# It4innovations/hyperqueue

Measured on AMD Instinct MI355X. Metric: tasks_assigned_per_sec, higher is better.
Workload: dtype u64

## Files before the change

hyperqueue_amd/csrc/debug_capi.cpp:

```cpp
#include "../../include/hqtick_debug.h"

#include <algorithm>
#include <cstring>

#include "hb_order.h"
#include "milp.h"
#include "price_emul.h"

static thread_local int g_last_canonical = 0;
static thread_local long g_last_hull[2] = {0, 0};
extern "C" int hqtick_debug_milp_was_canonical(void) { return g_last_canonical; }
extern "C" void hqtick_debug_milp_last_hull(long *solves, long *nonpacking) {
    if (solves) *solves = g_last_hull[0];
    if (nonpacking) *nonpacking = g_last_hull[1];
}

extern "C" int hqtick_debug_milp_solve(int ncols, const double *obj, const uint8_t *col_kind, int nrows, const uint8_t *row_type,
                                       const double *rhs, const int *row_off, const int *row_col, const double *row_coef,
                                       double time_limit_s, int canonical, double *x_out, double *obj_out, int *is_optimal,
                                       long *nodes_out) {
    hqmilp::Model m;
    m.obj.assign(obj, obj + ncols);
    m.kind.assign(col_kind, col_kind + ncols);
    m.rtype.assign(row_type, row_type + nrows);
// ... 27 lines not shown
    m.kind.assign(col_kind, col_kind + ncols);
    m.rtype.assign(row_type, row_type + nrows);
    m.rhs.assign(rhs, rhs + nrows);
    m.roff.assign(row_off, row_off + nrows + 1);
    int nnz = nrows ? row_off[nrows] : 0;
    m.rcol.assign(row_col, row_col + nnz);
    m.rcoef.assign(row_coef, row_coef + nnz);
    if (col_group) m.col_group.assign(col_group, col_group + ncols);
    if (row_implied) m.row_implied.assign(row_implied, row_implied + nrows);
    hqprice::EmulatedSweeper emu;
    if (min_cols) emu.min_cols = min_cols;
    hqmilp::Result r = hqmilp::solve(m, time_limit_s, true, hqmilp::REFERENCE_MIP_REL_GAP, use_sweeps ? &emu : nullptr);
    g_last_canonical = r.canonical ? 1 : 0;
    g_last_hull[0] = r.hull_solves; g_last_hull[1] = r.hull_solves_nonpacking;
    if (stats_out) { stats_out[0] = r.price_sweeps; stats_out[1] = r.price_rounds; stats_out[2] = r.price_total_us; stats_out[3] = r.canonical ? 1.0 : 0.0; }
    if (!r.feasible) return 0;
    for (int j = 0; j < ncols; j++) x_out[j] = r.x[j];
    *obj_out = r.objective;
    *is_optimal = r.optimal ? 1 : 0;
    return 1;
}

static thread_local hqmilp::Probe g_block_run_probe;
extern "C" void hqtick_debug_set_block_runs(int on) {
    hqmilp::g_probe = on < 0 ? nullptr : &g_block_run_probe; hqmilp::set_block_runs(on);
    if (on >= 0) { g_block_run_probe.model = g_block_run_probe.tables = g_block_run_probe.runs = g_block_run_probe.covered = 0; }
}
extern "C" void hqtick_debug_corrupt_block_runs(int on) { g_block_run_probe.corrupt_runs = on != 0; }
extern "C" void hqtick_debug_last_coupled_digest(uint64_t out[4]) {
    out[0] = g_block_run_probe.model; out[1] = g_block_run_probe.tables; out[2] = g_block_run_probe.runs; out[3] = g_block_run_probe.covered;
}
extern "C" void hqtick_debug_set_early_sweep(int on) { hqprice::set_early_sweep(on); }
extern "C" uint32_t hqtick_debug_early_sweeps(void) { return hqprice::early_sweeps(); }
extern "C" void hqtick_debug_capture_first_cut(int on) { hqprice::capture_first_cut(on != 0); }
extern "C" uint32_t hqtick_debug_first_cut(unsigned char *out, uint32_t cap) {
    const std::vector<unsigned char> &b = hqprice::first_cut_bytes();
    if (out && cap) memcpy(out, b.data(), std::min<size_t>(cap, b.size()));
    return (uint32_t)b.size();
}
```

hyperqueue_amd/csrc/hqtick.cpp:

```cpp
#include "../../include/hqtick.h"
#ifdef HQTICK_TEST_HOOKS
#include "../../include/hqtick_debug.h"
#endif

#include <dlfcn.h>
#include <hip/hip_runtime.h>
#include <rccl/rccl.h>

#include <algorithm>
#include <chrono>
#include <cstdio>
#include <cstdlib>
#include <cstring>
#include <functional>
#include <map>
#include <string>
#include <vector>

#include "block_solve.h"
#include "price_dev.h"
#ifdef HQTICK_TEST_HOOKS
#include "price_emul.h"
#endif
#include "devbuf.h"
// ... 2763 lines not shown
int hqtick_shard_allgather(hqtick_ctx *ctx, void *recv_device, size_t recv_bytes) {
    if (!ctx || !recv_device) return HQTICK_E_INVALID;
    if (!ctx->comm) return fail(ctx, HQTICK_E_INVALID, "hqtick_shard_allgather without hqtick_comm_init");
    if (!ctx->sink || !ctx->sink_bytes) return fail(ctx, HQTICK_E_INVALID, "hqtick_shard_allgather without a record sink (hqtick_set_record_sink)");
    if (recv_bytes < (size_t)ctx->comm_world * ctx->sink_bytes) return fail(ctx, HQTICK_E_CAPACITY, "receive buffer smaller than world x sink bytes");
    HQ_HIP(hipSetDevice(ctx->device));
    ncclResult_t rc = rccl().all_gather(ctx->sink, recv_device, ctx->sink_bytes, ncclUint8, ctx->comm, ctx->stream);
    if (rc != ncclSuccess) return fail(ctx, HQTICK_E_DEVICE, std::string("ncclAllGather: ") + rccl().err(rc));
    HQ_HIP(hipStreamSynchronize(ctx->stream));
    return 0;
}

}

namespace {
bool rccl_allgather_host(hqtick_ctx *ctx, const void *send, void *recv, size_t bytes) {
    if (!ctx->comm || bytes == 0) return false;
    const size_t total = bytes * ctx->comm_world;
    if (!ctx->h_xsend.ensure(bytes) || !ctx->h_xrecv.ensure(total) || !ctx->d_xsend.ensure(bytes) || !ctx->d_xrecv.ensure(total)) return false;
    if (hipSetDevice(ctx->device) != hipSuccess) return false;
    memcpy(ctx->h_xsend.p, send, bytes);
    if (hipMemcpyAsync(ctx->d_xsend.p, ctx->h_xsend.p, bytes, hipMemcpyHostToDevice, ctx->stream) != hipSuccess) return false;
    if (rccl().all_gather(ctx->d_xsend.p, ctx->d_xrecv.p, bytes, ncclUint8, ctx->comm, ctx->stream) != ncclSuccess) return false;
    if (hipMemcpyAsync(ctx->h_xrecv.p, ctx->d_xrecv.p, total, hipMemcpyDeviceToHost, ctx->stream) != hipSuccess) return false;
    if (hipStreamSynchronize(ctx->stream) != hipSuccess) return false;
    memcpy(recv, ctx->h_xrecv.p, total);
    return true;
}
}

extern "C" {

#ifdef HQTICK_TEST_HOOKS
int hqtick_debug_exchange(hqtick_ctx *ctx, const void *send, void *recv, size_t bytes_per_rank) {
    if (!ctx || !send || !recv) return HQTICK_E_INVALID;
    if (!ctx->comm) return fail(ctx, HQTICK_E_INVALID, "hqtick_debug_exchange without hqtick_comm_init");
    return rccl_allgather_host(ctx, send, recv, bytes_per_rank) ? 0 : fail(ctx, HQTICK_E_DEVICE, "the RCCL exchange failed");
}
#endif

int hqtick_comm_destroy(hqtick_ctx *ctx) {
    if (!ctx) return HQTICK_E_INVALID;
    if (ctx->comm) { hipSetDevice(ctx->device); rccl().destroy(ctx->comm); ctx->comm = nullptr; }
    ctx->comm_world = 0; ctx->comm_rank = 0;
    return 0;
}

}

static void rccl_destroy_comm(hqtick_ctx *ctx) { hqtick_comm_destroy(ctx); }
```

hyperqueue_amd/csrc/price.cpp:

```cpp
#include "price.h"

#include <algorithm>
#include <chrono>
#include <cmath>
#include <cstdio>
#include <cstdlib>
#include <cstring>
#include <functional>
#include <map>
#include <numeric>

#include "lp_tab.h"
#include "milp.h"

namespace hqprice {
namespace {

using hqmilp::lp::BASIC;
using hqmilp::lp::INF;
using hqmilp::lp::LP_OPT;
using hqmilp::lp::Rows;
using hqmilp::lp::Tab;

constexpr int KMAX_HOST = 128;
// ... 1624 lines not shown
            const uint32_t b = (uint32_t)P.block_of_flat[f];
            const double *ba = &bact[(size_t)b * MMAX_BLOCK];
            for (int r = 0; r < (int)T.blk_m[b] && step >= 1.0; r++) { const double a = T.col_a[(size_t)f * MMAX_BLOCK + r]; if (a > 0.0) { const double room = T.blk_cap[(size_t)b * MMAX_BLOCK + r] - ba[r]; if (room < a) { step = 0.0; break; } step = std::min(step, std::floor(room / a + 1e-9)); } }
            for (uint32_t e = T.col_woff[f]; e < T.col_woff[f + 1] && step >= 1.0; e++) {
                const double a = (double)T.w_coef[e];
                if (!(a > 0.0)) continue;
                const int g = T.w_row[e];
                for (int q = P.gr_off[g]; q < P.gr_off[g + 1]; q++) { const int k = P.gr_row[q]; const double room = P.h[k] - (ga[g] + fl[k]); if (room < 0.5 * a) { step = 0.0; break; } step = std::min(step, std::floor(room / a + 1e-9)); }
            }
            if (step < 1.0) continue;
            xf[f] += step;
            double *bw = &bact[(size_t)b * MMAX_BLOCK];
            for (int r = 0; r < MMAX_BLOCK; r++) bw[r] += T.col_a[(size_t)f * MMAX_BLOCK + r] * step;
            for (uint32_t e = T.col_woff[f]; e < T.col_woff[f + 1]; e++) ga[T.w_row[e]] += (double)T.w_coef[e] * step;
        }
        double z = 0.0;
        for (uint32_t f = 0; f < T.n_cols; f++) { x[P.model_of[f]] = xf[f]; z += T.col_cost[f] * xf[f]; }
        for (int g = 0; g < G; g++) z += P.gcost[g] * B[g];
        value = z;
        return true;
    }
};

}

Answer solve_model(const ModelView &mv, double rel_gap, double time_limit_s, double deadline_s, bool trace, Sweeper &sw, double *cost_scale) {
    const double tp0 = now_us();
    Request rq;
    rq.n = mv.n; rq.m = mv.m; rq.rel_gap = rel_gap; rq.time_limit_s = time_limit_s; rq.deadline_s = deadline_s; rq.trace = trace;
    Solver S(rq, sw);
    S.tp0 = tp0;
    if (g_capture_cut) g_first_cut.clear();
    std::vector<double> ub, c; double cmax = 1.0;
    const std::function<void()> hook = [&S]() { S.launch_on_blocks(); };
    if (const char *why = build_from_model(mv, S.P, ub, c, cmax, early_sweep_on() ? &hook : nullptr)) {
        if (S.early_begun) sw.end();
        Answer ans; ans.why = why; return ans;
    }
    if (cost_scale) *cost_scale = cmax;
    Polisher pol(S.P, mv.n);
    rq.polish = [&pol](std::vector<double> &x, double &value) { return pol.run(x, value); };
    return run_solver(S, tp0);
}

void flatten_for_probe(const ModelView &mv, bool trace) {
    Prob P; std::vector<double> ub, c; double cmax = 1.0;
    const char *why = build_from_model(mv, P, ub, c, cmax);
    if (trace) fprintf(stderr, "[price] flattened for the probe alone: %s\n", why ? why : "tables built");
}

void set_check_hints(bool on) { g_check_hints = on; g_hint_mismatches = 0; }
void set_early_sweep(int on) { g_early_sweep = on; g_early_sweeps = 0; }
uint32_t early_sweeps() { return g_early_sweeps; }
void capture_first_cut(bool on) { g_capture_cut = on; g_first_cut.clear(); }
const std::vector<unsigned char> &first_cut_bytes() { return g_first_cut; }
int hint_mismatches() { return g_hint_mismatches; }

Answer solve(const Request &rq, Sweeper &sw) {
    Solver S(rq, sw);
    const double tp0 = now_us();
    if (const char *why = build(rq, S.P)) { Answer ans; ans.why = why; return ans; }
    return run_solver(S, tp0);
}

}
```

hyperqueue_amd/csrc/price.h:

```cpp
#pragma once
#include <cstdint>
#include <functional>
#include <vector>

namespace hqprice {

struct HostTables {
    uint32_t n_blocks = 0, n_cols = 0, K = 0;
    std::vector<uint32_t> blk_off; std::vector<uint8_t> blk_m; std::vector<double> blk_cap;
    std::vector<double> col_cost, col_a; std::vector<int32_t> col_cap; std::vector<uint32_t> col_woff; std::vector<uint16_t> w_row; std::vector<int32_t> w_coef;
};

struct SweepTotals {
    double cx = 0, rc = 0, bnd = 0;
    uint32_t n_budget = 0, max_steps = 0;
    std::vector<long long> act;
    std::vector<double> part_cx;
    std::vector<long long> part_act;
};
constexpr int PARTS = 16;

struct RangeValues { const double *cx = nullptr, *rc = nullptr, *bnd = nullptr; const uint32_t *steps = nullptr; const long long *part_act = nullptr; };

void totals_from_blocks(uint32_t n_blocks, uint32_t K, const double *cx, const double *rc, const double *bnd, const uint32_t *steps, const long long *part_act, SweepTotals &out);
// ... 34 lines not shown
    std::function<bool(std::vector<double> &x, double &value)> polish;
    bool trace = false;
};

struct Answer {
    bool ran = false;
    double bound = 1e300;
    std::vector<double> x;
    double x_value = 0.0;
    uint32_t sweeps = 0, rounds = 0;
    const char *why = "";
    std::vector<int> block_of; std::vector<double> block_value, rcost;
};

Answer solve(const Request &rq, Sweeper &sw);

struct ModelView {
    int n = 0, m = 0;
    const double *obj = nullptr; const uint8_t *kind = nullptr;
    const uint8_t *rtype = nullptr; const double *rhs = nullptr;
    const int *roff = nullptr, *rcol = nullptr; const double *rcoef = nullptr;
    const int32_t *col_group = nullptr; const uint8_t *row_implied = nullptr;
    const int32_t *row_lhs = nullptr, *row_lhs_len = nullptr;
    const int *list_off = nullptr, *list_col = nullptr; int n_lists = 0;
    const int32_t *row_block = nullptr; const uint32_t *col_ub = nullptr;
    const int32_t *block_runs = nullptr; int n_block_runs = 0;
    uint64_t *run_stats = nullptr;
    uint64_t *tables_digest = nullptr;
};
void set_check_hints(bool on);
int hint_mismatches();
void set_early_sweep(int on);
uint32_t early_sweeps();
void capture_first_cut(bool on);
const std::vector<unsigned char> &first_cut_bytes();
void flatten_for_probe(const ModelView &mv, bool trace);
Answer solve_model(const ModelView &mv, double rel_gap, double time_limit_s, double deadline_s, bool trace, Sweeper &sw, double *cost_scale);

struct Exchange {
    uint32_t rank = 0, world = 1;
    virtual ~Exchange() {}
    virtual bool allgather(const void *send, void *recv, size_t bytes) = 0;
    uint64_t n_calls = 0, n_bytes = 0; double us = 0;
};

struct ShardedSweeper : Sweeper {
    Sweeper &inner; Exchange &ex;
    const HostTables *T = nullptr;
    std::vector<uint32_t> rank_b0, rank_b1, rank_p0, rank_p1;
    uint32_t max_blocks = 0, max_parts = 0, max_cols = 0;
    std::vector<unsigned char> send, recv;
    std::vector<double> cx, rc, bnd; std::vector<uint32_t> steps; std::vector<long long> part_act;
    std::vector<uint16_t> pats;
    uint32_t n_sweeps = 0;
    uint32_t min_blocks = 1025;
    bool pass = false;
    ShardedSweeper(Sweeper &in, Exchange &e, uint32_t min_blocks_) : inner(in), ex(e), min_blocks(min_blocks_) { min_cols = in.min_cols; budget = in.budget; }
    bool begin(const HostTables &t, uint32_t max_sweeps) override;
    bool set_caps(const int32_t *col_cap) override { return inner.set_caps(col_cap); }
    bool set_block_caps(const double *blk_cap) override { return inner.set_block_caps(blk_cap); }
    bool sweep(const double *pi, SweepTotals &out) override;
    const uint16_t *patterns(uint32_t first, uint32_t count) override;
    void end() override { inner.end(); T = nullptr; }
    bool merges_clock() const override { return ex.world > 1; }
};

// ... 2 lines not shown
```

hyperqueue_amd/csrc/price.hip:

```cpp
#include <hip/hip_runtime.h>

#include <algorithm>
#include <chrono>
#include <cstdio>
#include <cstdlib>
#include <cstring>
#include <type_traits>
#include <vector>

#include "dev_wave.h"
#include "price_core.h"
#include "price_dev.h"

namespace hqprice {

static_assert(PARTS == ASLOTS, "the master's parts are the kernel's activity slots");
constexpr int ASUB = 4;

namespace {

struct SweepResult {
    double cx, rc, bnd;
    uint32_t n_budget, max_steps;
    long long act[KMAX];
    double part_cx[ASLOTS];
    long long part_act[ASLOTS * KMAX];
    uint32_t seq;
};

struct PartVal { uint32_t nbud, mx; };

struct SweepArgs {
    Tables t;
    SweepOut out;
    uint32_t budget, seq;
    uint32_t *tickets;
    long long *tact;
    PartVal *pval;
    SweepResult *res;
    uint32_t first, local;
    double *lv_cx, *lv_rc, *lv_bnd; uint32_t *lv_steps;
    double pi[KMAX];
};

__device__ __forceinline__ double ld_dev(const double *p) { return __longlong_as_double((long long)__hip_atomic_load(reinterpret_cast<const unsigned long long *>(p), __ATOMIC_RELAXED, __HIP_MEMORY_SCOPE_AGENT)); }
__device__ __forceinline__ long long ld_dev(const long long *p) { return (long long)__hip_atomic_load(reinterpret_cast<const unsigned long long *>(p), __ATOMIC_RELAXED, __HIP_MEMORY_SCOPE_AGENT); }
__device__ __forceinline__ uint32_t ld_dev(const uint32_t *p) { return __hip_atomic_load(p, __ATOMIC_RELAXED, __HIP_MEMORY_SCOPE_AGENT); }
__device__ __forceinline__ void st_dev(long long *p, long long v) { __hip_atomic_store(reinterpret_cast<unsigned long long *>(p), (unsigned long long)v, __ATOMIC_RELAXED, __HIP_MEMORY_SCOPE_AGENT); }
__device__ __forceinline__ void st_dev(uint32_t *p, uint32_t v) { __hip_atomic_store(p, v, __ATOMIC_RELAXED, __HIP_MEMORY_SCOPE_AGENT); }
__device__ __forceinline__ void st_host(double *p, double v) { __hip_atomic_store(reinterpret_cast<unsigned long long *>(p), (unsigned long long)__double_as_longlong(v), __ATOMIC_RELAXED, __HIP_MEMORY_SCOPE_SYSTEM); }
__device__ __forceinline__ void st_host(long long *p, long long v) { __hip_atomic_store(reinterpret_cast<unsigned long long *>(p), (unsigned long long)v, __ATOMIC_RELAXED, __HIP_MEMORY_SCOPE_SYSTEM); }
__device__ __forceinline__ void st_host(uint32_t *p, uint32_t v) { __hip_atomic_store(p, v, __ATOMIC_RELAXED, __HIP_MEMORY_SCOPE_SYSTEM); }
__device__ __forceinline__ void acked() { __builtin_amdgcn_fence(__ATOMIC_RELEASE, "workgroup"); }

template <class SH, int NW>
__global__ __launch_bounds__(WAVE * NW) void k_price_sweep(const SweepArgs a) {
    __shared__ SH S;
    using WV = typename std::conditional<NW == 1, hqblock::DevWave, hqblock::DevGroup<NW>>::type;
    WV wv;
    if (NW > 1 && threadIdx.x >= WAVE) { hqblock::pool_helper(wv, S); return; }
    const uint32_t lane = threadIdx.x;
    const uint32_t nb = a.t.n_blocks, K = a.t.K, per = part_size(nb), b = a.first + blockIdx.x, p = b / per;
    solve_priced_block(wv, S, a.t, a.pi, b, a.out, a.budget);
    uint64_t *prof = a.out.prof ? a.out.prof + (size_t)b * PSLOTS : nullptr;
    const uint32_t r0 = a.first, r1 = a.first + gridDim.x;
    const uint32_t pb0 = p * per > r0 ? p * per : r0, pe = p * per + per < nb ? p * per + per : nb, pb1 = pe < r1 ? pe : r1;
    acked();
    if (prof && lane == 0) prof[11] = wv.now();
    uint32_t last = 0;
    if (lane == 0) last = __hip_atomic_fetch_add(&a.tickets[1 + p], 1u, __ATOMIC_RELAXED, __HIP_MEMORY_SCOPE_AGENT) == pb1 - pb0 - 1 ? 1u : 0u;
    last = (uint32_t)__builtin_amdgcn_readfirstlane((int)last);
    if (prof && lane == 0) prof[12] = wv.now();
    if (!last) return;
    {
        long long vs[2][ASUB];
#pragma unroll
        for (int u = 0; u < 2; u++) {
            const uint32_t k = lane + (uint32_t)u * WAVE;
#pragma unroll
            for (int sub = 0; sub < ASUB; sub++) vs[u][sub] = k < K ? ld_dev(&a.out.act[((size_t)p * ASUB + sub) * K + k]) : 0;
        }
        double *scr = &S.py[0][0];
        static_assert(sizeof(S.py) >= 256 * sizeof(double), "a round of the part's c.x values is staged in the dual pool's storage");
        uint32_t nbud = 0, mx = 0;
        double s4 = 0.0;
        for (uint32_t c0 = p * per; c0 < pe; c0 += 256) {
            double v[4]; uint32_t vst[4];
#pragma unroll
            for (int u = 0; u < 4; u++) { const uint32_t q = c0 + lane + (uint32_t)u * WAVE; v[u] = (q < pe && !a.local) ? ld_dev(&a.out.blk_cx[q]) : 0.0; vst[u] = (q >= pb0 && q < pb1) ? ld_dev(&a.out.blk_steps[q]) : 0u; }
#pragma unroll
            for (int u = 0; u < 4; u++) { scr[lane + (uint32_t)u * WAVE] = v[u]; nbud += vst[u] >> 31; const uint32_t st = vst[u] & 0x7FFFFFFFu; mx = st > mx ? st : mx; }
            wv.sync();
            const uint32_t cnt = pe - c0 < 256u ? pe - c0 : 256u;
            if (lane < 4 && !a.local) for (uint32_t i = lane; i < cnt; i += 4) s4 += scr[i];
            wv.sync();
        }
// ... 71 lines not shown
    if (lane == 0) __hip_atomic_store(&a.res->seq, a.seq, __ATOMIC_RELEASE, __HIP_MEMORY_SCOPE_SYSTEM);
}

constexpr size_t SYNC_ACT = 128, SYNC_PACT = SYNC_ACT + (size_t)ASLOTS * ASUB * KMAX * 8, SYNC_PVAL = SYNC_PACT + (size_t)KMAX * 8, SYNC_BYTES = SYNC_PVAL + (size_t)ASLOTS * sizeof(PartVal);

constexpr int NPROF = 13;
const int PROF_FROM[NPROF] = {0, 1, 3, 4, 5, 5, 8, 9, 10, 6, 11, 12, 13};
const int PROF_TO[NPROF]   = {1, 2, 4, 5, 6, 8, 9, 10, 6, 11, 12, 13, 14};
const char *const PROF_NAME[NPROF] = {"reduced costs + compaction", "dual pool + order + greedy fills", "level lists + root bound", "walk", "results + activities", "[results: zero the sums", "pattern + sums in LDS", "atomics + cost loads", "values]",
                                      "acknowledgements before the ticket", "part ticket", "part sums + sweep ticket + totals (last block)", "system fence (last block)"};

size_t al16(size_t v) { return (v + 15) & ~(size_t)15; }
double now_us() { return std::chrono::duration<double, std::micro>(std::chrono::steady_clock::now().time_since_epoch()).count(); }

}

DeviceSweeper::~DeviceSweeper() { h_stage.release(); h_res.release(); h_pats.release(); h_pin.release(); h_blkv.release(); d_tab.release(); d_pats.release(); d_blk.release(); d_sync.release(); d_prof.release(); }

bool DeviceSweeper::size_buffers(const HostTables &t, uint32_t max_sweeps) {
    if (profile && (!h_prof.ensure((size_t)t.n_blocks * PSLOTS * 8 + 64) || !d_prof.ensure((size_t)t.n_blocks * PSLOTS * 8 + 64))) return false;
    T = &t; n_sweeps = 0; cap_sweeps = max_sweeps; blocks_only = false;
    max_block_cols = 0;
    for (uint32_t b = 0; b < t.n_blocks; b++) max_block_cols = std::max(max_block_cols, t.blk_off[b + 1] - t.blk_off[b]);
    if (force_nmax) max_block_cols = (uint32_t)hqblock::NMAX;
    o_off = 0; o_m = al16(o_off + (size_t)(t.n_blocks + 1) * 4); o_cap = al16(o_m + t.n_blocks); o_cost = al16(o_cap + (size_t)t.n_blocks * MMAX * 8);
    o_a = al16(o_cost + (size_t)t.n_cols * 8); o_ccap = al16(o_a + (size_t)t.n_cols * MMAX * 8); o_woff = al16(o_ccap + (size_t)t.n_cols * 4);
    o_wrow = al16(o_woff + (size_t)(t.n_cols + 1) * 4);
    if (!h_res.ensure(sizeof(SweepResult) + 64)) return false;
    if (!h_pin.ensure((size_t)std::min<uint32_t>(max_sweeps, PIN_SWEEPS) * t.n_cols * 2 + 64)) return false;
    in_flight = false;
    return d_pats.ensure((size_t)max_sweeps * t.n_cols * 2) && d_blk.ensure((size_t)t.n_blocks * 28 + 64) && d_sync.ensure(SYNC_BYTES);
}

void DeviceSweeper::stage_blocks(const HostTables &t) {
    unsigned char *h = h_stage.as<unsigned char>();
    memcpy(h + o_off, t.blk_off.data(), (size_t)(t.n_blocks + 1) * 4); memcpy(h + o_m, t.blk_m.data(), t.n_blocks); memcpy(h + o_cap, t.blk_cap.data(), (size_t)t.n_blocks * MMAX * 8);
    memcpy(h + o_cost, t.col_cost.data(), (size_t)t.n_cols * 8); memcpy(h + o_a, t.col_a.data(), (size_t)t.n_cols * MMAX * 8); memcpy(h + o_ccap, t.col_cap.data(), (size_t)t.n_cols * 4);
}

bool DeviceSweeper::begin(const HostTables &t, uint32_t max_sweeps) {
    if (t.K > (uint32_t)KMAX || t.n_blocks == 0) return false;
    if (!size_buffers(t, max_sweeps)) return false;
    const size_t nw = t.w_row.size();
    wide_room = std::max(wide_room, nw);
    o_wcoef = al16(o_wrow + nw * 2); tab_bytes = al16(o_wcoef + nw * 4);
    if (!h_stage.ensure(tab_bytes) || !d_tab.ensure(tab_bytes)) return false;
    unsigned char *h = h_stage.as<unsigned char>();
    stage_blocks(t);
    memcpy(h + o_woff, t.col_woff.data(), (size_t)(t.n_cols + 1) * 4);
    if (nw) { memcpy(h + o_wrow, t.w_row.data(), nw * 2); memcpy(h + o_wcoef, t.w_coef.data(), nw * 4); }
    if (hipMemcpyAsync(d_tab.p, h, tab_bytes, hipMemcpyHostToDevice, stream) != hipSuccess) return false;
    if (!sync_clean) { if (hipMemsetAsync(d_sync.p, 0, SYNC_BYTES, stream) != hipSuccess) return false; }
    SweepResult *r = h_res.as<SweepResult>();
    seq = r->seq;
    return true;
}

int DeviceSweeper::begin_blocks(const HostTables &t, uint32_t max_sweeps) {
    if (t.n_blocks == 0 || !size_buffers(t, max_sweeps)) return 0;
    const size_t room = std::max(wide_room, (size_t)t.n_cols * 4);
    o_wcoef = o_wrow; tab_bytes = o_wrow;
    const size_t dev_bytes = al16(al16(o_wrow + room * 2) + room * 4);
    if (!h_stage.ensure(o_wrow + (dev_bytes - o_woff)) || !d_tab.ensure(dev_bytes)) return 0;
    unsigned char *h = h_stage.as<unsigned char>();
    stage_blocks(t);
    memset(h + o_woff, 0, o_wrow - o_woff);
    if (hipMemcpyAsync(d_tab.p, h, o_wrow, hipMemcpyHostToDevice, stream) != hipSuccess) return 0;
    if (!sync_clean) { if (hipMemsetAsync(d_sync.p, 0, SYNC_BYTES, stream) != hipSuccess) return 0; }
    seq = h_res.as<SweepResult>()->seq;
    blocks_only = true;
    return 1;
}

bool DeviceSweeper::begin_wide() {
    if (!T || !blocks_only) return false;
    const HostTables &t = *T;
    if (t.K > (uint32_t)KMAX || t.col_woff.size() != (size_t)t.n_cols + 1) return false;
    const size_t nw = t.w_row.size();
    wide_room = std::max(wide_room, nw);
    o_wcoef = al16(o_wrow + nw * 2); tab_bytes = al16(o_wcoef + nw * 4);
    const size_t wide_bytes = tab_bytes - o_woff;
    if (o_wrow + wide_bytes > h_stage.cap || tab_bytes > d_tab.cap) {
        if (hipStreamSynchronize(stream) != hipSuccess) return false;
        if (!h_stage.ensure(o_wrow + wide_bytes) || !d_tab.ensure(tab_bytes)) return false;
        unsigned char *h = h_stage.as<unsigned char>();
        stage_blocks(t);
        memcpy(h + o_woff, t.col_woff.data(), (size_t)(t.n_cols + 1) * 4);
        if (nw) { memcpy(h + o_wrow, t.w_row.data(), nw * 2); memcpy(h + o_wcoef, t.w_coef.data(), nw * 4); }
        if (hipMemcpyAsync(d_tab.p, h, tab_bytes, hipMemcpyHostToDevice, stream) != hipSuccess) return false;
    } else {
        unsigned char *h = h_stage.as<unsigned char>() + o_wrow;
        memcpy(h, t.col_woff.data(), (size_t)(t.n_cols + 1) * 4);
        if (nw) { memcpy(h + (o_wrow - o_woff), t.w_row.data(), nw * 2); memcpy(h + (o_wcoef - o_woff), t.w_coef.data(), nw * 4); }
        if (hipMemcpyAsync(d_tab.as<unsigned char>() + o_woff, h, wide_bytes, hipMemcpyHostToDevice, stream) != hipSuccess) return false;
    }
    blocks_only = false;
    return true;
}

bool DeviceSweeper::set_caps(const int32_t *col_cap) {
    if (!T) return false;
    memcpy(h_stage.as<unsigned char>() + o_ccap, col_cap, (size_t)T->n_cols * 4);
    return hipMemcpyAsync(d_tab.as<unsigned char>() + o_ccap, h_stage.as<unsigned char>() + o_ccap, (size_t)T->n_cols * 4, hipMemcpyHostToDevice, stream) == hipSuccess;
}

bool DeviceSweeper::set_block_caps(const double *blk_cap) {
    if (!T) return false;
    const size_t bytes = (size_t)T->n_blocks * MMAX * 8;
    memcpy(h_stage.as<unsigned char>() + o_cap, blk_cap, bytes);
    return hipMemcpyAsync(d_tab.as<unsigned char>() + o_cap, h_stage.as<unsigned char>() + o_cap, bytes, hipMemcpyHostToDevice, stream) == hipSuccess;
}

bool DeviceSweeper::sweep(const double *pi, SweepTotals &out) { return launch(pi, 0, T ? T->n_blocks : 0, false, &out); }

bool DeviceSweeper::sweep_range(const double *pi, uint32_t b0, uint32_t b1, RangeValues &rv) {
    if (!T || b1 > T->n_blocks || b0 > b1) return false;
    const uint32_t nb = T->n_blocks;
    if (!h_blkv.ensure((size_t)nb * 28 + 64)) return false;
    if (b1 > b0) { if (!launch(pi, b0, b1, true, nullptr)) return false; }
    else {
        if (n_sweeps >= cap_sweeps) return false;
        SweepResult *r = h_res.as<SweepResult>();
        memset(r->part_act, 0, sizeof(r->part_act));
        n_sweeps++;
    }
    unsigned char *h = h_blkv.as<unsigned char>();
    rv = RangeValues{(const double *)h, (const double *)(h + (size_t)nb * 8), (const double *)(h + (size_t)nb * 16), (const uint32_t *)(h + (size_t)nb * 24), h_res.as<SweepResult>()->part_act};
    return true;
}

bool DeviceSweeper::launch(const double *pi, uint32_t b0, uint32_t b1, bool local, SweepTotals *outp) { return launch_only(pi, b0, b1, local) && wait_done(outp); }
bool DeviceSweeper::sweep_launch(const double *pi) { return launch_only(pi, 0, T ? T->n_blocks : 0, false); }
bool DeviceSweeper::sweep_finish(SweepTotals &out) { return wait_done(&out); }

bool DeviceSweeper::launch_only(const double *pi, uint32_t b0, uint32_t b1, bool local) {
    if (!T || n_sweeps >= cap_sweeps || b1 <= b0 || in_flight) return false;
    if (blocks_only && (n_sweeps != 0 || local)) return false;
    const HostTables &t = *T;
    const uint32_t K = blocks_only ? 0u : t.K;
    unsigned char *d = d_tab.as<unsigned char>();
    SweepArgs a;
    a.t = Tables{t.n_blocks, t.n_cols, K, (const uint32_t *)(d + o_off), (const uint8_t *)(d + o_m), (const double *)(d + o_cap), (const double *)(d + o_cost), (const double *)(d + o_a),
                 (const int32_t *)(d + o_ccap), (const uint32_t *)(d + o_woff), (const uint16_t *)(d + o_wrow), (const int32_t *)(d + o_wcoef)};
    unsigned char *blk = d_blk.as<unsigned char>();
    uint16_t *xdst = n_sweeps < PIN_SWEEPS ? h_pin.dev<uint16_t>() + (size_t)n_sweeps * t.n_cols : d_pats.as<uint16_t>() + (size_t)n_sweeps * t.n_cols;
    a.out = SweepOut{xdst, (double *)blk, (double *)(blk + (size_t)t.n_blocks * 8), (double *)(blk + (size_t)t.n_blocks * 16),
                     (long long *)(d_sync.as<unsigned char>() + SYNC_ACT), (uint32_t *)(blk + (size_t)t.n_blocks * 24), profile ? d_prof.as<uint64_t>() : nullptr, (uint32_t)ASUB, dbg};
    a.budget = budget; a.seq = ++seq; a.tickets = d_sync.as<uint32_t>(); a.tact = (long long *)(d_sync.as<unsigned char>() + SYNC_PACT); a.pval = (PartVal *)(d_sync.as<unsigned char>() + SYNC_PVAL); a.res = h_res.dev<SweepResult>();
    a.first = b0; a.local = local ? 1u : 0u;
    if (local) { unsigned char *lv = h_blkv.dev<unsigned char>(); a.lv_cx = (double *)lv; a.lv_rc = (double *)(lv + (size_t)t.n_blocks * 8); a.lv_bnd = (double *)(lv + (size_t)t.n_blocks * 16); a.lv_steps = (uint32_t *)(lv + (size_t)t.n_blocks * 24); }
    else { a.lv_cx = a.lv_rc = a.lv_bnd = nullptr; a.lv_steps = nullptr; }
    memset(a.pi, 0, sizeof(a.pi));
    if (K) memcpy(a.pi, pi, (size_t)K * 8);
    const double t0 = now_us();
    const uint32_t nblk = b1 - b0;
    const int nw = force_waves == 1 || force_waves == 2 ? force_waves : 4;
#define HQ_SWEEP(SH_, NW_) hipLaunchKernelGGL((k_price_sweep<SH_, NW_>), dim3(nblk), dim3(WAVE * NW_), 0, stream, a)
#define HQ_SWEEP_N(SH_) do { if (nw == 4) HQ_SWEEP(SH_, 4); else if (nw == 2) HQ_SWEEP(SH_, 2); else HQ_SWEEP(SH_, 1); } while (0)
    if (max_block_cols <= 8) HQ_SWEEP_N(hqblock::SharedN<8>);
    else if (max_block_cols <= 16) HQ_SWEEP_N(hqblock::SharedN<16>);
    else HQ_SWEEP_N(hqblock::SharedN<hqblock::NMAX>);
#undef HQ_SWEEP_N
#undef HQ_SWEEP
    if (hipGetLastError() != hipSuccess) return false;
    in_flight = true; sync_clean = false; flight_t0 = t0; flight_blocks = b1 - b0; flight_k = K;
    return true;
}

bool DeviceSweeper::wait_done(SweepTotals *outp) {
    if (!T || !in_flight) return false;
    in_flight = false;
    const HostTables &t = *T;
    const double t0 = flight_t0;
    volatile SweepResult *r = h_res.as<SweepResult>();
    for (uint64_t spins = 0;; spins++) {
        if (__atomic_load_n(&r->seq, __ATOMIC_ACQUIRE) == seq) break;
        if ((spins & 0xFFFF) == 0xFFFF && now_us() - t0 > 2.0e6) {
            if (hipStreamSynchronize(stream) != hipSuccess) return false;
            if (__atomic_load_n(&r->seq, __ATOMIC_ACQUIRE) != seq) return false;
            break;
        }
    }
    last_kernel_us = now_us() - t0;
    sync_clean = true;
    if (profile) {
        if (hipMemcpyAsync(h_prof.p, d_prof.p, (size_t)t.n_blocks * PSLOTS * 8, hipMemcpyDeviceToHost, stream) != hipSuccess || hipStreamSynchronize(stream) != hipSuccess) return false;
        const uint64_t *pr = h_prof.as<uint64_t>();
        for (int st = 0; st < NPROF; st++) {
            const int from = PROF_FROM[st], to = PROF_TO[st];
            std::vector<double> v; v.reserve(t.n_blocks);
// ... 16 lines not shown
    out.act.resize(K);
    for (uint32_t k = 0; k < K; k++) out.act[k] = r->act[k];
    out.part_cx.assign(r->part_cx, r->part_cx + ASLOTS);
    out.part_act.resize((size_t)ASLOTS * K);
    for (size_t i = 0; i < (size_t)ASLOTS * K; i++) out.part_act[i] = r->part_act[i];
    return true;
}

const uint16_t *DeviceSweeper::patterns(uint32_t first, uint32_t count) {
    if (!T || first + count > n_sweeps || in_flight) return nullptr;
    const size_t nc = T->n_cols, bytes = (size_t)count * nc * 2;
    if (first + count <= PIN_SWEEPS) return h_pin.as<uint16_t>() + (size_t)first * nc;
    if (!h_pats.ensure(bytes + 64)) return nullptr;
    if (count == 0) return h_pats.as<uint16_t>();
    const uint32_t n_pin = first < PIN_SWEEPS ? PIN_SWEEPS - first : 0;
    if (n_pin) memcpy(h_pats.p, h_pin.as<uint16_t>() + (size_t)first * nc, (size_t)n_pin * nc * 2);
    if (hipMemcpyAsync(h_pats.as<uint16_t>() + (size_t)n_pin * nc, d_pats.as<uint16_t>() + (size_t)(first + n_pin) * nc, bytes - (size_t)n_pin * nc * 2, hipMemcpyDeviceToHost, stream) != hipSuccess) return nullptr;
    if (hipStreamSynchronize(stream) != hipSuccess) return nullptr;
    return h_pats.as<uint16_t>();
}

void DeviceSweeper::end() {
    if (in_flight) { hipStreamSynchronize(stream); in_flight = false; }
    if (profile && prof_n) {
        fprintf(stderr, "[price profile] %d sweeps, per block and sweep (us; median over blocks / slowest block, averaged over the sweeps):", prof_n);
        for (int st = 0; st < NPROF; st++) fprintf(stderr, "  %s %.1f / %.1f;", PROF_NAME[st], prof_med[st] / prof_n, prof_max[st] / prof_n);
        fprintf(stderr, "  first block's start -> last block's results %.1f, -> completion word stored %.1f more;", prof_span / prof_n, prof_tail / prof_n);
        fprintf(stderr, "  most search steps of a block %.0f; sweep as the host saw it %.1f us\n", prof_steps / prof_n, total_us / (double)std::max<uint64_t>(1, total_sweeps));
        for (int st = 0; st < NPROF; st++) prof_med[st] = prof_max[st] = 0; prof_steps = 0; prof_span = prof_tail = 0; prof_n = 0;
    }
    T = nullptr; blocks_only = false;
}

}
```

hyperqueue_amd/csrc/price_dev.h:

```cpp
#pragma once
#include <hip/hip_runtime.h>

#include <cstdlib>

#include "devbuf.h"
#include "price.h"

namespace hqprice {

struct DeviceSweeper : Sweeper {
    hipStream_t stream = nullptr;
    hqbuf::PinBuf h_stage, h_res, h_pats, h_pin, h_prof, h_blkv;
    static constexpr uint32_t PIN_SWEEPS = 64;
    bool sync_clean = false;
    bool in_flight = false; double flight_t0 = 0; uint32_t flight_blocks = 0;
    bool profile = getenv("HQTICK_PRICE_PROFILE") != nullptr; double prof_med[16] = {0}, prof_max[16] = {0}, prof_steps = 0, prof_span = 0, prof_tail = 0; int prof_n = 0;
    hqbuf::DevBuf d_tab, d_pats, d_blk, d_sync, d_prof;
    const HostTables *T = nullptr;
    size_t o_off = 0, o_m = 0, o_cap = 0, o_cost = 0, o_a = 0, o_ccap = 0, o_woff = 0, o_wrow = 0, o_wcoef = 0, tab_bytes = 0;
    bool blocks_only = false;
    uint32_t flight_k = 0;
    size_t wide_room = 0;
    uint32_t n_sweeps = 0, cap_sweeps = 0, seq = 0;
    uint32_t max_block_cols = 0;
    bool force_nmax = getenv("HQTICK_PRICE_NMAX") != nullptr;
    int force_waves = getenv("HQTICK_PRICE_WAVES") ? atoi(getenv("HQTICK_PRICE_WAVES")) : 0;
    uint32_t dbg = getenv("HQTICK_PRICE_DBG") ? (uint32_t)atoi(getenv("HQTICK_PRICE_DBG")) : 0u;
    double last_kernel_us = 0;
    uint64_t total_sweeps = 0, total_block_solves = 0; double total_us = 0;
    explicit DeviceSweeper(hipStream_t s) : stream(s) {}
    ~DeviceSweeper() override;
    bool begin(const HostTables &t, uint32_t max_sweeps) override;
    int begin_blocks(const HostTables &t, uint32_t max_sweeps) override;
    bool begin_wide() override;
    bool size_buffers(const HostTables &t, uint32_t max_sweeps);
    void stage_blocks(const HostTables &t);
    bool set_caps(const int32_t *col_cap) override;
    bool set_block_caps(const double *blk_cap) override;
    bool sweep(const double *pi, SweepTotals &out) override;
    bool sweep_range(const double *pi, uint32_t b0, uint32_t b1, RangeValues &out) override;
    bool launch(const double *pi, uint32_t b0, uint32_t b1, bool local, SweepTotals *out);
    bool launch_only(const double *pi, uint32_t b0, uint32_t b1, bool local);
    bool wait_done(SweepTotals *out);
    bool sweep_launch(const double *pi) override;
    bool sweep_finish(SweepTotals &out) override;
    const uint16_t *patterns(uint32_t first, uint32_t count) override;
    void end() override;
};

}
```

include/hqtick_debug.h:

```cpp
#ifndef HQTICK_DEBUG_H
#define HQTICK_DEBUG_H
#include <stdint.h>
#include "hqtick.h"
#ifdef __cplusplus
extern "C" {
#endif
#if defined(__GNUC__)
#pragma GCC visibility push(default)
#endif

int hqtick_debug_milp_solve(int ncols, const double *obj, const uint8_t *col_kind, int nrows, const uint8_t *row_type,
                            const double *rhs, const int *row_off, const int *row_col, const double *row_coef,
                            double time_limit_s, int canonical, double *x_out, double *obj_out, int *is_optimal,
                            long *nodes_out);

int hqtick_debug_last_order(const hqtick_ctx *ctx, uint32_t *n_runs, uint32_t *n_levels, double *order_us);

int hqtick_debug_last_scan(const hqtick_ctx *ctx, int which, uint32_t *n_levels, uint32_t *n_groups, uint32_t shape[4],
                           uint64_t *levels, uint32_t cap_levels, uint32_t *hist, uint32_t cap_groups);

int hqtick_debug_host_stages(const hqtick_config *config, const hqtick_snapshot *snapshot, const uint8_t *vflags, const uint32_t *vtmc,
                             uint32_t n_levels, const uint64_t *levels, const uint32_t *hist, hqtick_result *out);

int hqtick_debug_host_query(const hqtick_config *config, const hqtick_snapshot *snapshot, const hqtick_query_workers *fake,
                            const uint8_t *vflags, const uint32_t *vtmc, const uint8_t *fake_vflags, const uint32_t *fake_vtmc,
                            uint32_t n_levels, const uint64_t *levels, const uint32_t *hist, hqtick_query_result *out);

int hqtick_debug_milp_was_canonical(void);
void hqtick_debug_milp_last_hull(long *solves, long *nonpacking);

void hqtick_debug_map_order_u32(const uint32_t *keys, uint32_t n, uint32_t *out_pos);

int hqtick_debug_block_solve_host(uint32_t n_cols, uint32_t n_resources, const uint32_t *ent_off, const uint32_t *ent_res, const uint8_t *ent_kind,
                                  const uint64_t *ent_amount, const uint32_t *weight, const double *pool, uint32_t n_classes, const uint64_t *free_,
                                  const uint64_t *total, const uint64_t *elig, uint32_t budget, uint32_t *x, uint32_t *status, uint32_t *steps);
void hqtick_debug_set_block_emulation(int on, uint32_t budget);
void hqtick_debug_last_stage_us(double *out3);
void hqtick_debug_last_blocks(uint32_t *n_emulated, uint32_t *n_host);

int hqtick_time_kernel(hqtick_ctx *ctx, int which, int iters, double *avg_us);
int hqtick_timeline(const hqtick_ctx *ctx, double *out, int cap);
const uint64_t *hqtick_block_profile_last(const hqtick_ctx *ctx, uint32_t *n_classes);


void hqtick_debug_set_price_emulation(int on, uint32_t min_cols);
void hqtick_debug_set_price_fault(int fail_at);
void hqtick_debug_set_fast_path(int on);
void hqtick_debug_check_model_hints(int on);
int hqtick_debug_model_hint_mismatches(void);
void hqtick_debug_set_block_runs(int on);
void hqtick_debug_last_coupled_digest(uint64_t out[4]);
void hqtick_debug_set_early_sweep(int on);
uint32_t hqtick_debug_early_sweeps(void);
void hqtick_debug_capture_first_cut(int on);
uint32_t hqtick_debug_first_cut(unsigned char *out, uint32_t cap);
void hqtick_debug_corrupt_block_runs(int on);
void hqtick_debug_last_price(uint32_t *sweeps, uint32_t *rounds);
uint32_t hqtick_debug_last_mn(const uint32_t **rq, const uint32_t **off, const uint32_t **worker);
int hqtick_debug_milp_solve_priced(int ncols, const double *obj, const uint8_t *col_kind, const int32_t *col_group, int nrows, const uint8_t *row_type,
                                   const uint8_t *row_implied, const double *rhs, const int *row_off, const int *row_col, const double *row_coef,
                                   double time_limit_s, int use_sweeps, uint32_t min_cols, double *x_out, double *obj_out, int *is_optimal, double *stats_out);

struct hqwire_tables;
struct hqwire_records;
struct hqwire_output;
int hqwire_debug_encode_host(const struct hqwire_tables *tables, const struct hqwire_records *records, const struct hqwire_output *out);
int hqwire_debug_encode_host_order(const struct hqwire_tables *tables, const struct hqwire_records *records, const struct hqwire_output *out, int order);

void hqtick_debug_set_block_guard(uint32_t verify, uint32_t tick_seq, int corrupt_mode, uint32_t corrupt_class, uint32_t corrupt_fill);
void hqtick_debug_last_block_guard(uint32_t *verified, uint32_t *mismatch, uint32_t *rejected);
void hqtick_debug_set_block_memo(int on);
uint32_t hqtick_debug_last_block_memo(void);
void hqtick_debug_set_exchange(hqtick_exchange_fn fn, void *user, uint32_t rank, uint32_t world, uint32_t min_blocks, uint32_t min_classes);
uint32_t hqtick_debug_last_exchange_calls(void);
int hqtick_debug_exchange(hqtick_ctx *ctx, const void *send, void *recv, size_t bytes_per_rank);
#if defined(__GNUC__)
#pragma GCC visibility pop
#endif
#ifdef __cplusplus
}
#endif
#endif
```

Before: 69.46 million.

## Read first blocks-only sweep from pinned staging and write tables through to device

For the blocks-only first sweep, the explicit host-to-device copy of the block tables is now skipped by default. The kernel instead reads the tables directly from the pinned host staging buffer, and each block writes its slice (plus the padding gaps) through to the device table buffer. The aim is to overlap the table upload with the first sweep rather than waiting on a separate memcpy. The cost is slower host-memory reads during that sweep and extra kernel work, plus new debug hooks (an env toggle and a device-vs-host table digest) to check that the device copy ends up consistent.

```diff
diff --git a/hyperqueue_amd/csrc/debug_capi.cpp b/hyperqueue_amd/csrc/debug_capi.cpp
--- a/hyperqueue_amd/csrc/debug_capi.cpp
+++ b/hyperqueue_amd/csrc/debug_capi.cpp
@@ -83,6 +83,7 @@
 }
 extern "C" void hqtick_debug_set_early_sweep(int on) { hqprice::set_early_sweep(on); }
 extern "C" uint32_t hqtick_debug_early_sweeps(void) { return hqprice::early_sweeps(); }
+extern "C" void hqtick_debug_set_first_sweep_copy(int on) { hqprice::set_first_sweep_copy(on); }
 extern "C" void hqtick_debug_capture_first_cut(int on) { hqprice::capture_first_cut(on != 0); }
 extern "C" uint32_t hqtick_debug_first_cut(unsigned char *out, uint32_t cap) {
     const std::vector<unsigned char> &b = hqprice::first_cut_bytes();
diff --git a/hyperqueue_amd/csrc/hqtick.cpp b/hyperqueue_amd/csrc/hqtick.cpp
--- a/hyperqueue_amd/csrc/hqtick.cpp
+++ b/hyperqueue_amd/csrc/hqtick.cpp
@@ -2819,6 +2819,12 @@
 extern "C" {
 
 #ifdef HQTICK_TEST_HOOKS
+int hqtick_debug_device_tables_digest(hqtick_ctx *ctx, uint64_t out[3]) {
+    if (!ctx || !out) return HQTICK_E_INVALID;
+    if (!ctx->pricer) return fail(ctx, HQTICK_E_INVALID, "hqtick_debug_device_tables_digest: the context has no device sweeper");
+    if (hipSetDevice(ctx->device) != hipSuccess) return fail(ctx, HQTICK_E_DEVICE, "hipSetDevice failed");
+    return ctx->pricer->tables_digest(&out[0], &out[1], &out[2]) ? 0 : fail(ctx, HQTICK_E_INVALID, "hqtick_debug_device_tables_digest: no coupled solve has left its tables on the device");
+}
 int hqtick_debug_exchange(hqtick_ctx *ctx, const void *send, void *recv, size_t bytes_per_rank) {
     if (!ctx || !send || !recv) return HQTICK_E_INVALID;
     if (!ctx->comm) return fail(ctx, HQTICK_E_INVALID, "hqtick_debug_exchange without hqtick_comm_init");
diff --git a/hyperqueue_amd/csrc/price.cpp b/hyperqueue_amd/csrc/price.cpp
--- a/hyperqueue_amd/csrc/price.cpp
+++ b/hyperqueue_amd/csrc/price.cpp
@@ -1680,8 +1680,12 @@
     S.tp0 = tp0;
     if (g_capture_cut) g_first_cut.clear();
     std::vector<double> ub, c; double cmax = 1.0;
-    const std::function<void()> hook = [&S]() { S.launch_on_blocks(); };
-    if (const char *why = build_from_model(mv, S.P, ub, c, cmax, early_sweep_on() ? &hook : nullptr)) {
+    const bool early = early_sweep_on();
+    const std::function<void()> hook = [&S, early, trace, tp0]() {
+        if (trace) fprintf(stderr, "[price] block tables final at %.3f ms\n", (now_us() - tp0) / 1e3);
+        if (early) S.launch_on_blocks();
+    };
+    if (const char *why = build_from_model(mv, S.P, ub, c, cmax, &hook)) {
         if (S.early_begun) sw.end();
         Answer ans; ans.why = why; return ans;
     }
@@ -1699,6 +1703,12 @@
 
 void set_check_hints(bool on) { g_check_hints = on; g_hint_mismatches = 0; }
 void set_early_sweep(int on) { g_early_sweep = on; g_early_sweeps = 0; }
+static thread_local int g_first_sweep_copy = -1;
+void set_first_sweep_copy(int on) { g_first_sweep_copy = on; }
+bool first_sweep_copy_on() {
+    static const bool env_on = getenv("HQPRICE_FIRST_SWEEP_COPY") && atoi(getenv("HQPRICE_FIRST_SWEEP_COPY")) != 0;
+    return g_first_sweep_copy < 0 ? env_on : g_first_sweep_copy != 0;
+}
 uint32_t early_sweeps() { return g_early_sweeps; }
 void capture_first_cut(bool on) { g_capture_cut = on; g_first_cut.clear(); }
 const std::vector<unsigned char> &first_cut_bytes() { return g_first_cut; }
diff --git a/hyperqueue_amd/csrc/price.h b/hyperqueue_amd/csrc/price.h
--- a/hyperqueue_amd/csrc/price.h
+++ b/hyperqueue_amd/csrc/price.h
@@ -90,6 +90,8 @@
 int hint_mismatches();
 void set_early_sweep(int on);
 uint32_t early_sweeps();
+void set_first_sweep_copy(int on);
+bool first_sweep_copy_on();
 void capture_first_cut(bool on);
 const std::vector<unsigned char> &first_cut_bytes();
 void flatten_for_probe(const ModelView &mv, bool trace);
diff --git a/hyperqueue_amd/csrc/price.hip b/hyperqueue_amd/csrc/price.hip
--- a/hyperqueue_amd/csrc/price.hip
+++ b/hyperqueue_amd/csrc/price.hip
@@ -40,6 +40,7 @@
     SweepResult *res;
     uint32_t first, local;
     double *lv_cx, *lv_rc, *lv_bnd; uint32_t *lv_steps;
+    long long wt_delta;
     double pi[KMAX];
 };
 
@@ -53,15 +54,57 @@
 __device__ __forceinline__ void st_host(uint32_t *p, uint32_t v) { __hip_atomic_store(p, v, __ATOMIC_RELAXED, __HIP_MEMORY_SCOPE_SYSTEM); }
 __device__ __forceinline__ void acked() { __builtin_amdgcn_fence(__ATOMIC_RELEASE, "workgroup"); }
 
-template <class SH, int NW>
+template <class T> __device__ __forceinline__ T *wt_ptr(const T *src, long long delta) { return reinterpret_cast<T *>(reinterpret_cast<uintptr_t>(src) + (uintptr_t)delta); }
+__device__ __forceinline__ void wt_gap(const void *end, const void *next, long long d, uint32_t lane) {
+    const unsigned char *s = static_cast<const unsigned char *>(end);
+    const size_t n = (size_t)(static_cast<const unsigned char *>(next) - s);
+    if (lane < n && n < 16) wt_ptr(s, d)[lane] = s[lane];
+}
+__device__ void write_through(const Tables &t, long long d, uint32_t b, uint32_t lane) {
+    const uint32_t c0 = t.blk_off[b], c1 = t.blk_off[b + 1], nc = c1 - c0;
+    if (c1 < c0 || c1 > t.n_cols) return;
+    const uint8_t m = t.blk_m[b];
+    const double cap = lane < (uint32_t)MMAX ? t.blk_cap[(size_t)b * MMAX + lane] : 0.0;
+    for (uint32_t i0 = 0; i0 < nc; i0 += WAVE) {
+        const uint32_t i = i0 + lane;
+        const bool in = i < nc;
+        const size_t j = (size_t)c0 + i;
+        const double cost = in ? t.col_cost[j] : 0.0;
+        const int32_t ccap = in ? t.col_cap[j] : 0;
+        double av[MMAX];
+#pragma unroll
+        for (int r = 0; r < MMAX; r++) av[r] = in ? t.col_a[j * MMAX + r] : 0.0;
+        if (in) {
+            wt_ptr(t.col_cost, d)[j] = cost;
+            wt_ptr(t.col_cap, d)[j] = ccap;
+            wt_ptr(t.col_woff, d)[j] = 0u;
+#pragma unroll
+            for (int r = 0; r < MMAX; r++) wt_ptr(t.col_a, d)[j * MMAX + r] = av[r];
+        }
+    }
+    if (lane < (uint32_t)MMAX) wt_ptr(t.blk_cap, d)[(size_t)b * MMAX + lane] = cap;
+    if (lane == 0) { wt_ptr(t.blk_off, d)[b] = c0; wt_ptr(t.blk_off, d)[b + 1] = c1; wt_ptr(t.blk_m, d)[b] = m; wt_ptr(t.col_woff, d)[c1] = 0u; }
+    if (b == 0) {
+        wt_gap(t.blk_off + t.n_blocks + 1, t.blk_m, d, lane); wt_gap(t.blk_m + t.n_blocks, t.blk_cap, d, lane); wt_gap(t.blk_cap + (size_t)t.n_blocks * MMAX, t.col_cost, d, lane);
+        wt_gap(t.col_cost + t.n_cols, t.col_a, d, lane); wt_gap(t.col_a + (size_t)t.n_cols * MMAX, t.col_cap, d, lane); wt_gap(t.col_cap + t.n_cols, t.col_woff, d, lane);
+        wt_gap(t.col_woff + t.n_cols + 1, t.w_row, d, lane);
+    }
+}
+
+template <class SH, int NW, bool WT>
 __global__ __launch_bounds__(WAVE * NW) void k_price_sweep(const SweepArgs a) {
     __shared__ SH S;
     using WV = typename std::conditional<NW == 1, hqblock::DevWave, hqblock::DevGroup<NW>>::type;
     WV wv;
-    if (NW > 1 && threadIdx.x >= WAVE) { hqblock::pool_helper(wv, S); return; }
+    if (NW > 1 && threadIdx.x >= WAVE) {
+        hqblock::pool_helper(wv, S);
+        if (WT && threadIdx.x >= (uint32_t)WAVE * (NW - 1)) write_through(a.t, a.wt_delta, a.first + blockIdx.x, threadIdx.x & (uint32_t)(WAVE - 1));
+        return;
+    }
     const uint32_t lane = threadIdx.x;
     const uint32_t nb = a.t.n_blocks, K = a.t.K, per = part_size(nb), b = a.first + blockIdx.x, p = b / per;
     solve_priced_block(wv, S, a.t, a.pi, b, a.out, a.budget);
+    if (WT && NW == 1) write_through(a.t, a.wt_delta, b, lane);
     uint64_t *prof = a.out.prof ? a.out.prof + (size_t)b * PSLOTS : nullptr;
     const uint32_t r0 = a.first, r1 = a.first + gridDim.x;
     const uint32_t pb0 = p * per > r0 ? p * per : r0, pe = p * per + per < nb ? p * per + per : nb, pb1 = pe < r1 ? pe : r1;
@@ -199,15 +242,23 @@
     return d_pats.ensure((size_t)max_sweeps * t.n_cols * 2) && d_blk.ensure((size_t)t.n_blocks * 28 + 64) && d_sync.ensure(SYNC_BYTES);
 }
 
+static void zero_gap(unsigned char *h, size_t end, size_t next) { if (next > end) memset(h + end, 0, next - end); }
+
 void DeviceSweeper::stage_blocks(const HostTables &t) {
     unsigned char *h = h_stage.as<unsigned char>();
     memcpy(h + o_off, t.blk_off.data(), (size_t)(t.n_blocks + 1) * 4); memcpy(h + o_m, t.blk_m.data(), t.n_blocks); memcpy(h + o_cap, t.blk_cap.data(), (size_t)t.n_blocks * MMAX * 8);
     memcpy(h + o_cost, t.col_cost.data(), (size_t)t.n_cols * 8); memcpy(h + o_a, t.col_a.data(), (size_t)t.n_cols * MMAX * 8); memcpy(h + o_ccap, t.col_cap.data(), (size_t)t.n_cols * 4);
+    zero_gap(h, o_off + (size_t)(t.n_blocks + 1) * 4, o_m); zero_gap(h, o_m + t.n_blocks, o_cap); zero_gap(h, o_cap + (size_t)t.n_blocks * MMAX * 8, o_cost);
+    zero_gap(h, o_cost + (size_t)t.n_cols * 8, o_a); zero_gap(h, o_a + (size_t)t.n_cols * MMAX * 8, o_ccap); zero_gap(h, o_ccap + (size_t)t.n_cols * 4, o_woff);
+}
+void DeviceSweeper::zero_wide_gaps(unsigned char *h, size_t n_cols, size_t nw) {
+    zero_gap(h, (n_cols + 1) * 4, o_wrow - o_woff); zero_gap(h, o_wrow - o_woff + nw * 2, o_wcoef - o_woff); zero_gap(h, o_wcoef - o_woff + nw * 4, tab_bytes - o_woff);
 }
 
 bool DeviceSweeper::begin(const HostTables &t, uint32_t max_sweeps) {
     if (t.K > (uint32_t)KMAX || t.n_blocks == 0) return false;
     if (!size_buffers(t, max_sweeps)) return false;
+    from_stage = false; wide_behind = false;
     const size_t nw = t.w_row.size();
     wide_room = std::max(wide_room, nw);
     o_wcoef = al16(o_wrow + nw * 2); tab_bytes = al16(o_wcoef + nw * 4);
@@ -216,6 +267,7 @@
     stage_blocks(t);
     memcpy(h + o_woff, t.col_woff.data(), (size_t)(t.n_cols + 1) * 4);
     if (nw) { memcpy(h + o_wrow, t.w_row.data(), nw * 2); memcpy(h + o_wcoef, t.w_coef.data(), nw * 4); }
+    zero_wide_gaps(h + o_woff, t.n_cols, nw);
     if (hipMemcpyAsync(d_tab.p, h, tab_bytes, hipMemcpyHostToDevice, stream) != hipSuccess) return false;
     if (!sync_clean) { if (hipMemsetAsync(d_sync.p, 0, SYNC_BYTES, stream) != hipSuccess) return false; }
     SweepResult *r = h_res.as<SweepResult>();
@@ -232,10 +284,11 @@
     unsigned char *h = h_stage.as<unsigned char>();
     stage_blocks(t);
     memset(h + o_woff, 0, o_wrow - o_woff);
-    if (hipMemcpyAsync(d_tab.p, h, o_wrow, hipMemcpyHostToDevice, stream) != hipSuccess) return 0;
+    from_stage = !first_sweep_copy_on();
+    if (!from_stage && hipMemcpyAsync(d_tab.p, h, o_wrow, hipMemcpyHostToDevice, stream) != hipSuccess) return 0;
     if (!sync_clean) { if (hipMemsetAsync(d_sync.p, 0, SYNC_BYTES, stream) != hipSuccess) return 0; }
     seq = h_res.as<SweepResult>()->seq;
-    blocks_only = true;
+    blocks_only = true; wide_behind = false;
     return 1;
 }
 
@@ -254,12 +307,15 @@
         stage_blocks(t);
         memcpy(h + o_woff, t.col_woff.data(), (size_t)(t.n_cols + 1) * 4);
         if (nw) { memcpy(h + o_wrow, t.w_row.data(), nw * 2); memcpy(h + o_wcoef, t.w_coef.data(), nw * 4); }
+        zero_wide_gaps(h + o_woff, t.n_cols, nw);
         if (hipMemcpyAsync(d_tab.p, h, tab_bytes, hipMemcpyHostToDevice, stream) != hipSuccess) return false;
     } else {
         unsigned char *h = h_stage.as<unsigned char>() + o_wrow;
         memcpy(h, t.col_woff.data(), (size_t)(t.n_cols + 1) * 4);
         if (nw) { memcpy(h + (o_wrow - o_woff), t.w_row.data(), nw * 2); memcpy(h + (o_wcoef - o_woff), t.w_coef.data(), nw * 4); }
+        zero_wide_gaps(h, t.n_cols, nw);
         if (hipMemcpyAsync(d_tab.as<unsigned char>() + o_woff, h, wide_bytes, hipMemcpyHostToDevice, stream) != hipSuccess) return false;
+        wide_behind = true;
     }
     blocks_only = false;
     return true;
@@ -305,8 +361,10 @@
     if (blocks_only && (n_sweeps != 0 || local)) return false;
     const HostTables &t = *T;
     const uint32_t K = blocks_only ? 0u : t.K;
-    unsigned char *d = d_tab.as<unsigned char>();
+    const bool wt = blocks_only && from_stage;
+    unsigned char *d = wt ? h_stage.dev<unsigned char>() : d_tab.as<unsigned char>();
     SweepArgs a;
+    a.wt_delta = wt ? (long long)((uintptr_t)d_tab.p - (uintptr_t)d) : 0;
     a.t = Tables{t.n_blocks, t.n_cols, K, (const uint32_t *)(d + o_off), (const uint8_t *)(d + o_m), (const double *)(d + o_cap), (const double *)(d + o_cost), (const double *)(d + o_a),
                  (const int32_t *)(d + o_ccap), (const uint32_t *)(d + o_woff), (const uint16_t *)(d + o_wrow), (const int32_t *)(d + o_wcoef)};
     unsigned char *blk = d_blk.as<unsigned char>();
@@ -322,7 +380,7 @@
     const double t0 = now_us();
     const uint32_t nblk = b1 - b0;
     const int nw = force_waves == 1 || force_waves == 2 ? force_waves : 4;
-#define HQ_SWEEP(SH_, NW_) hipLaunchKernelGGL((k_price_sweep<SH_, NW_>), dim3(nblk), dim3(WAVE * NW_), 0, stream, a)
+#define HQ_SWEEP(SH_, NW_) do { if (wt) hipLaunchKernelGGL((k_price_sweep<SH_, NW_, true>), dim3(nblk), dim3(WAVE * NW_), 0, stream, a); else hipLaunchKernelGGL((k_price_sweep<SH_, NW_, false>), dim3(nblk), dim3(WAVE * NW_), 0, stream, a); } while (0)
 #define HQ_SWEEP_N(SH_) do { if (nw == 4) HQ_SWEEP(SH_, 4); else if (nw == 2) HQ_SWEEP(SH_, 2); else HQ_SWEEP(SH_, 1); } while (0)
     if (max_block_cols <= 8) HQ_SWEEP_N(hqblock::SharedN<8>);
     else if (max_block_cols <= 16) HQ_SWEEP_N(hqblock::SharedN<16>);
@@ -405,4 +463,17 @@
     T = nullptr; blocks_only = false;
 }
 
-}
+bool DeviceSweeper::tables_digest(uint64_t *dev, uint64_t *host, uint64_t *bytes) {
+    if (in_flight || blocks_only || tab_bytes == 0 || tab_bytes > d_tab.cap || o_woff > tab_bytes) return false;
+    std::vector<unsigned char> back(tab_bytes);
+    if (hipMemcpyAsync(back.data(), d_tab.p, tab_bytes, hipMemcpyDeviceToHost, stream) != hipSuccess || hipStreamSynchronize(stream) != hipSuccess) return false;
+    auto fnv = [](uint64_t h, const unsigned char *p, size_t n) { for (size_t i = 0; i < n; i++) { h ^= p[i]; h *= 1099511628211ull; } return h; };
+    const uint64_t seed = 14695981039346656037ull;
+    const unsigned char *h = h_stage.as<unsigned char>();
+    *dev = fnv(seed, back.data(), tab_bytes);
+    *host = wide_behind ? fnv(fnv(seed, h, o_woff), h + o_wrow, tab_bytes - o_woff) : fnv(seed, h, tab_bytes);
+    *bytes = tab_bytes;
+    return true;
+}
+
+}
diff --git a/hyperqueue_amd/csrc/price_dev.h b/hyperqueue_amd/csrc/price_dev.h
--- a/hyperqueue_amd/csrc/price_dev.h
+++ b/hyperqueue_amd/csrc/price_dev.h
@@ -19,6 +19,8 @@
     const HostTables *T = nullptr;
     size_t o_off = 0, o_m = 0, o_cap = 0, o_cost = 0, o_a = 0, o_ccap = 0, o_woff = 0, o_wrow = 0, o_wcoef = 0, tab_bytes = 0;
     bool blocks_only = false;
+    bool from_stage = false;
+    bool wide_behind = false;
     uint32_t flight_k = 0;
     size_t wide_room = 0;
     uint32_t n_sweeps = 0, cap_sweeps = 0, seq = 0;
@@ -35,6 +37,7 @@
     bool begin_wide() override;
     bool size_buffers(const HostTables &t, uint32_t max_sweeps);
     void stage_blocks(const HostTables &t);
+    void zero_wide_gaps(unsigned char *h, size_t n_cols, size_t nw);
     bool set_caps(const int32_t *col_cap) override;
     bool set_block_caps(const double *blk_cap) override;
     bool sweep(const double *pi, SweepTotals &out) override;
@@ -46,6 +49,7 @@
     bool sweep_finish(SweepTotals &out) override;
     const uint16_t *patterns(uint32_t first, uint32_t count) override;
     void end() override;
+    bool tables_digest(uint64_t *dev, uint64_t *host, uint64_t *bytes);
 };
 
 }
diff --git a/include/hqtick_debug.h b/include/hqtick_debug.h
--- a/include/hqtick_debug.h
+++ b/include/hqtick_debug.h
@@ -52,6 +52,8 @@
 void hqtick_debug_last_coupled_digest(uint64_t out[4]);
 void hqtick_debug_set_early_sweep(int on);
 uint32_t hqtick_debug_early_sweeps(void);
+void hqtick_debug_set_first_sweep_copy(int on);
+int hqtick_debug_device_tables_digest(hqtick_ctx *ctx, uint64_t out[3]);
 void hqtick_debug_capture_first_cut(int on);
 uint32_t hqtick_debug_first_cut(unsigned char *out, uint32_t cap);
 void hqtick_debug_corrupt_block_runs(int on);
```

Measured after the change: 74.59 million (median of 6 runs). 7.4% higher.
